# guanlongzhao/fac-via-ppg

Measured on AMD Instinct MI355X. Metric: 22.05 kHz audio samples/sec end-to-end PPG→wav; real-time factor at batch=1, higher is better.
Workload: dtype f32

## Files before the change

### fac-via-ppg_amd/csrc/facppg_taco.hip

```cpp

#include <algorithm>
#include <cstdlib>
#include <cstring>
#include <mutex>
#include <new>

#include "facppg_gemm.h"

using namespace facppg;

struct facppg_taco {
  facppg_taco_config c;
  int device;
  int coop_limit;
  int wall_khz;
  char* arena;
  float4 *pre0, *pre1, *conv[8], *wih;
  float *conv_b[8], *conv_scale[8], *conv_shift[8];
  float *whh_t[2], *lstm_b;
  float4* mem_w;
  float *dp0_t, *dp1_t, *att_t, *att_b, *dec_t, *dec_b, *q_t, *proj_t, *proj_b;
  float *loc_conv, *loc_dense, *v;
  float *att_coop[5], *dec_coop[5];
  int coop_U[5], coop_nwg[5];
// ... 976 lines not shown
  if (tid < U && unit0 + tid < A) {
    const float* gs = part + 4 * NT;
    const float h = lstm_point(gs[tid], gs[U + tid], gs[2 * U + tid], gs[3 * U + tid], &cstate[tid]);
    __hip_atomic_store(xchg_out + unit0 + tid, ((unsigned long long)tag << 32) | __float_as_uint(h), __ATOMIC_RELAXED,
                       __HIP_MEMORY_SCOPE_AGENT);
  }
}

template <int NT>
__device__ __forceinline__ void coop_gather(const unsigned long long* xchg, unsigned tag, int n, float* dst0, float* dst1, int tid) {
  for (int i = tid; i < n; i += NT) {
    const float h = __uint_as_float((unsigned)poll_tag(xchg + i, tag));
    dst0[i] = h; dst1[i] = h;
  }
  __syncthreads();
}

__global__ __launch_bounds__(NTC) void k_decoder_coop(DecArgs p) {
  extern __shared__ float sm[];
  __shared__ int s_stop;
  __shared__ float c_att[160], c_dec[160];
  const int wg = blockIdx.x, b = p.b0 + blockIdx.y, tid = threadIdx.x;
  const bool leader = wg == 0;
  const int len = p.lengths ? p.lengths[b] : p.Tin;
  DecLds L;
  dec_carve(p, sm, L);
  dec_init<NTC>(p, L, sm, tid);
  if (tid == 0) s_stop = 0;
  if (tid < 160) { c_att[tid] = 0.0f; c_dec[tid] = 0.0f; }
  __syncthreads();
  const float* mem = p.memory + (size_t)b * p.Tin * p.E;
  const float* pm = p.pm + (size_t)b * p.Tin * p.AD;
  float* ah = L.in_att + p.P + p.E;
  float* dh = L.in_dec + p.A + p.E;
  unsigned long long* xa = p.xchg + (size_t)b * 2 * p.A;
  unsigned long long* xd = xa + p.A;
  const int SC = 4 * p.U, unit0 = wg * p.U;
  const float* att_slice = p.att_coop + (size_t)wg * L.KA * SC;
  const float* dec_slice = p.dec_coop + (size_t)wg * L.KD * SC;
  long long tk = clock64();
#define PROF(slot)                                                        \
  if (p.prof && leader && b == 0 && tid == 0) {                           \
    const long long now = clock64();                                      \
    p.prof[slot] += now - tk;                                             \
    tk = now;                                                             \
  }
  for (int t = 0;; ++t) {
    if (t > 0) {
      dec_project<NTC>(p, L, t - 1, b, tid, leader, &s_stop);
      if (s_stop) {
        if (leader && tid == 0) p.out_len[b] = t;
        break;
      }
    }
    PROF(0)
    dec_prenet<NTC>(p, L, t, b, tid);
    PROF(1)
    coop_lstm_slice<NTC>(att_slice, p.att_b, L.KA, p.U, p.A, unit0, L.in_att, L.part, c_att, xa, t + 1, tid);
    PROF(2)
    coop_gather<NTC>(xa, t + 1, p.A, ah, L.in_dec, tid);
    PROF(3)
    PROF(4)
    dec_attention<NTC>(p, L, mem, pm, len, t, b, tid, leader);
    PROF(5)
    coop_lstm_slice<NTC>(dec_slice, p.dec_b, L.KD, p.U, p.D, unit0, L.in_dec, L.part, c_dec, xd, t + 1, tid);
    PROF(6)
    coop_gather<NTC>(xd, t + 1, p.D, dh, L.in_proj, tid);
    PROF(7)
  }
#undef PROF
}

constexpr int SU = 4, SSC = 4 * SU, SKP = NTC / SSC;
constexpr int SKR_LSTM = 40, SKR_PROJ = 32, SKR_P1 = 4, SKR_P2 = 12;

__device__ __forceinline__ void xpub(unsigned long long* w, float v, unsigned tag) {
  __hip_atomic_store(w, ((unsigned long long)tag << 32) | __float_as_uint(v), __ATOMIC_RELAXED, __HIP_MEMORY_SCOPE_AGENT);
}
__device__ __forceinline__ float xwait(const unsigned long long* w, unsigned tag) {
  return __uint_as_float((unsigned)poll_tag(w, tag));
}

template <int KRM>
__device__ __forceinline__ void stat_load(float (&w)[KRM], const float* __restrict__ W, int ld, int row0, int nrows, int K, int tid) {
  const int r = tid % SSC, kp = tid / SSC, KR = (K + SKP - 1) / SKP;
#pragma unroll
  for (int i = 0; i < KRM; ++i) {
    const int k = kp * KR + i;
    w[i] = (i < KR && k < K && row0 + r < nrows) ? W[(size_t)k * ld + row0 + r] : 0.0f;
  }
}
template <int KRM>
__device__ __forceinline__ void stat_mv16(const float (&w)[KRM], int K, const float* in, float* part, int tid) {
  const int r = tid % SSC, kp = tid / SSC, KR = (K + SKP - 1) / SKP;
  const int kb = kp * KR;
  float acc = 0.0f;
#pragma unroll
  for (int i = 0; i < KRM; ++i) acc = fmaf(w[i], in[kb + i], acc);
  acc += __shfl_xor(acc, 16);
  acc += __shfl_xor(acc, 32);
  if ((tid & 63) < SSC) part[(tid >> 6) * SSC + r] = acc;
  __syncthreads();
  if (tid < SSC) {
    float s = 0.0f;
#pragma unroll
    for (int j = 0; j < NTC / 64; ++j) s += part[j * SSC + tid];
    part[256 + tid] = s;
  }
  __syncthreads();
}

constexpr int SNU = 4;

template <int KRM, int NU>
__device__ __forceinline__ void stat_mv16n(const float (&w)[KRM], int K, const float* in0, int ustride, unsigned alive, float* part,
                                           int tid) {
  if constexpr (NU > 2) {
#pragma unroll
    for (int u = 0; u < NU; ++u)
      if (alive >> u & 1) {
        stat_mv16(w, K, in0 + (size_t)u * ustride, part, tid);
        if (tid < SSC) part[512 + u * SSC + tid] = part[256 + tid];
      }
    return;
  }
  const int r = tid % SSC, kp = tid / SSC, KR = (K + SKP - 1) / SKP;
  const int kb = kp * KR;
  float acc[NU];
#pragma unroll
  for (int u = 0; u < NU; ++u) acc[u] = 0.0f;
#pragma unroll
  for (int i = 0; i < KRM; ++i)
#pragma unroll
    for (int u = 0; u < NU; ++u) acc[u] = fmaf(w[i], in0[(size_t)u * ustride + kb + i], acc[u]);
#pragma unroll
  for (int u = 0; u < NU; ++u) {
    acc[u] += __shfl_xor(acc[u], 16);
    acc[u] += __shfl_xor(acc[u], 32);
    if ((tid & 63) < SSC) part[((tid >> 6) * NU + u) * SSC + r] = acc[u];
  }
  __syncthreads();
  if (tid < SSC * NU) {
    const int u = tid / SSC, rr = tid % SSC;
    float s = 0.0f;
#pragma unroll
    for (int j = 0; j < NTC / 64; ++j) s += part[(j * NU + u) * SSC + rr];
    part[512 + tid] = s;
  }
  __syncthreads();
  (void)alive;
}

template <int NU>
__global__ __launch_bounds__(NTC) void k_decoder_split(DecArgs p) {
  extern __shared__ float sm[];
  __shared__ int s_stop[SNU];
  __shared__ float c_att[SNU][SU], c_dec[SNU][SU];
  const int blk = blockIdx.x, grp = blockIdx.y, tid = threadIdx.x;
  const size_t xstride = (size_t)(p.NF + 1 + 2 * p.P + p.A + p.E + p.D + 8);
  const int KA = p.P + p.E + p.A, KD = p.A + p.E + p.D, KP = p.D + p.E;
  if (tid < SNU) s_stop[tid] = 0;
  if (blk >= NU) {
    const int wg = blk - NU, unit0 = wg * SU, row0 = wg * SSC;
    const int ustride = KA + KD + KP + round_up(p.NF, 4) + round_up(p.P, 4);
    float* part = sm + (size_t)NU * ustride;
    for (int i = tid; i < NU * ustride + 1024; i += NTC) sm[i] = 0.0f;
    if (tid < SNU * SU) { (&c_att[0][0])[tid] = 0.0f; (&c_dec[0][0])[tid] = 0.0f; }
    float w_att[SKR_LSTM], w_dec[SKR_LSTM], w_proj[SKR_PROJ], w_p1[SKR_PROJ], w_p2[SKR_P2];
    stat_load(w_att, p.att_w4 + (size_t)wg * KA * SSC, SSC, 0, SSC, KA, tid);
    stat_load(w_dec, p.dec_w4 + (size_t)wg * KD * SSC, SSC, 0, SSC, KD, tid);
    const int pre_wk = (p.P + SSC - 1) / SSC, proj_wk = (p.NF + 1 + SSC - 1) / SSC;
    const int proj_w0 = pre_wk + proj_wk <= p.nwk ? pre_wk : 0;
    const int prow0 = (wg - proj_w0) * SSC;
    stat_load(w_proj, p.proj_t, round_up(p.NF + 1, 4), prow0 < 0 ? p.NF + 1 : prow0, p.NF + 1, KP, tid);
    stat_load(w_p1, p.w1p_t, round_up(p.P, 4), row0, p.P, KP, tid);
    stat_load(w_p2, p.dp1_t, round_up(p.P, 4), row0, p.P, p.P, tid);
    const bool has_proj = prow0 >= 0 && prow0 < p.NF + 1, has_pre = row0 < p.P;
    unsigned alive = 0;
    for (int u = 0; u < NU; ++u)
      if (grp * NU + u < p.B) alive |= 1u << u;
    __syncthreads();
#define FOR_ALIVE(u) _Pragma("unroll") for (int u = 0; u < NU; ++u) if (alive >> u & 1)
#define UTT(u)                                                                                          \
  const int b = grp * NU + u;                                                                           \
  unsigned long long* MEL = p.xsplit + (size_t)b * xstride;                                             \
  unsigned long long *X1 = MEL + p.NF + 1, *X2 = X1 + p.P, *AH = X2 + p.P, *CTX = AH + p.A, *DH = CTX + p.E; \
  float* in_att = sm + (size_t)u * ustride; float* in_dec = in_att + KA; float* in_proj = in_dec + KD;  \
  float* xin = in_proj + KP; float* p1 = xin + round_up(p.NF, 4);                                       \
  (void)MEL; (void)X1; (void)X2; (void)AH; (void)CTX; (void)DH; (void)in_att; (void)in_dec; (void)in_proj; (void)xin; (void)p1
    long long wtk = clock64();
#define WPROF(slot)                                                       \
  if (p.prof && wg == 0 && grp == 0 && tid == 0) {                        \
    const long long now = clock64();                                      \
    p.prof[16 + slot] += now - wtk;                                       \
    wtk = now;                                                            \
  }
    for (int t = 0;; ++t) {
      const unsigned tag = t + 1;
      if (t > 0) {
        if (has_proj) stat_mv16n<SKR_PROJ, NU>(w_proj, KP, sm + KA + KD, ustride, alive, part, tid);
        if (has_proj) FOR_ALIVE(u) {
          UTT(u);
          if (tid < SSC && prow0 + tid <= p.NF) {
            const int row = prow0 + tid;
            const float v = part[512 + u * SSC + tid] + p.proj_b[row];
            if (row < p.NF) {
              p.mel[((size_t)b * p.NF + row) * p.max_steps + t - 1] = v;
              if (p.melx) xpub(p.melx + (size_t)(t - 1) * p.NF + row, v, tag - 1);
            } else { p.gate[(size_t)b * p.max_steps + t - 1] = v; xpub(MEL + row, v, tag); }
          }
        }
        if (has_pre) stat_mv16n<SKR_PROJ, NU>(w_p1, KP, sm + KA + KD, ustride, alive, part, tid);
        if (has_pre) FOR_ALIVE(u) {
          UTT(u);
          const uint8_t* mk = p.masks + ((size_t)t * 2 * p.B + b) * p.P;
          if (tid < SSC && row0 + tid < p.P)
            xpub(X1 + row0 + tid, fmaxf(part[512 + u * SSC + tid] + p.b1p[row0 + tid], 0.0f) * (float)mk[row0 + tid] * 2.0f, tag);
        }
        WPROF(0)
        FOR_ALIVE(u) {
          UTT(u);
          if (tid == 0) s_stop[u] = sigm(xwait(MEL + p.NF, tag)) > p.gate_thr || t == dec_step_limit(p, b);
        }
        __syncthreads();
        for (int u = 0; u < NU; ++u)
          if (s_stop[u]) alive &= ~(1u << u);
        if (!alive) break;
        FOR_ALIVE(u) {
          UTT(u);
          for (int i = tid; i < p.P; i += NTC) p1[i] = xwait(X1 + i, tag);
        }
        __syncthreads();
        WPROF(1)
      }
      if (has_pre) stat_mv16n<SKR_P2, NU>(w_p2, p.P, sm + KA + KD + KP + round_up(p.NF, 4), ustride, alive, part, tid);
      if (has_pre) FOR_ALIVE(u) {
        UTT(u);
        const uint8_t* mk = p.masks + ((size_t)t * 2 * p.B + b) * p.P;
        if (tid < SSC && row0 + tid < p.P)
          xpub(X2 + row0 + tid, fmaxf(part[512 + u * SSC + tid], 0.0f) * (float)mk[(size_t)p.B * p.P + row0 + tid] * 2.0f, tag);
      }
      WPROF(2)
      FOR_ALIVE(u) {
        UTT(u);
        for (int i = tid; i < p.P; i += NTC) in_att[i] = xwait(X2 + i, tag);
// ... 271 lines not shown
  auto take = [&](size_t bytes) { size_t o = off; off += (bytes + 255) / 256 * 256; return o; };
  const size_t E = c.encoder_embedding_dim > c.symbols_embedding_dim ? c.encoder_embedding_dim : c.symbols_embedding_dim;
  w.a0 = take((size_t)B * E * Tin * 4);
  w.a1 = take((size_t)B * E * Tin * 4);
  w.xproj = take((size_t)B * Tin * 4 * c.encoder_embedding_dim * 4);
  w.mem_cm = take((size_t)B * c.encoder_embedding_dim * Tin * 4);
  w.mask = take((size_t)2 * B * c.symbols_embedding_dim * Tin);
  w.xchg = take((size_t)B * 2 * 2 * (c.encoder_embedding_dim / 2) * 8);
  const size_t mx = c.encoder_embedding_dim > c.symbols_embedding_dim ? c.encoder_embedding_dim : c.symbols_embedding_dim;
  w.splitk_bytes = (size_t)16 * B * mx * Tin * 4;
  w.splitk = take(w.splitk_bytes);
  w.total = off;
  return w;
}

}

static int taco_check(const facppg_taco_config* c) {
  FACPPG_REQUIRE(c, FACPPG_EINVAL, "config is NULL");
  FACPPG_REQUIRE(c->n_symbols > 0 && c->symbols_embedding_dim > 0 && c->encoder_embedding_dim > 0 && c->encoder_embedding_dim % 2 == 0,
                 FACPPG_EINVAL, "bad encoder dims");
  FACPPG_REQUIRE(c->symbols_embedding_dim == c->encoder_embedding_dim, FACPPG_EUNSUPPORTED,
                 "symbols_embedding_dim must equal encoder_embedding_dim (prenet feeds the conv bank)");
  FACPPG_REQUIRE(c->encoder_n_convolutions >= 0 && c->encoder_n_convolutions <= 8 && c->postnet_n_convolutions >= 2 &&
                     c->postnet_n_convolutions <= 8 && c->encoder_kernel_size % 2 == 1 && c->postnet_kernel_size % 2 == 1,
                 FACPPG_EUNSUPPORTED, "conv stack sizes out of range");
  FACPPG_REQUIRE(c->attention_rnn_dim == c->decoder_rnn_dim && c->attention_rnn_dim % 4 == 0 && 4 * c->attention_rnn_dim <= 4096,
                 FACPPG_EUNSUPPORTED, "attention_rnn_dim must equal decoder_rnn_dim, be a multiple of 4 and <= 1024");
  FACPPG_REQUIRE(c->attention_location_n_filters >= 1 && c->attention_location_n_filters <= 32 && c->attention_dim >= 1 &&
                     c->attention_dim <= 256,
                 FACPPG_EUNSUPPORTED, "attention_location_n_filters must be <= 32 and attention_dim <= 256 (one MFMA pass each)");
  FACPPG_REQUIRE(c->encoder_embedding_dim <= 768 && c->prenet_dim <= NTC && c->attention_dim <= NTC && c->n_acoustic_feat_dims < NTC &&
                     (2 * c->encoder_embedding_dim) % 4 == 0,
                 FACPPG_EUNSUPPORTED, "decoder dims exceed the 512-thread cooperative workgroup");
  FACPPG_REQUIRE(c->attention_location_kernel_size % 2 == 1 && c->attention_location_n_filters > 0, FACPPG_EUNSUPPORTED,
                 "attention_location_kernel_size must be odd");
  return FACPPG_OK;
}

static size_t taco_count(const facppg_taco_config* c) {
  const size_t S = c->symbols_embedding_dim, E = c->encoder_embedding_dim, H = E / 2, K = c->encoder_kernel_size;
  const size_t P = c->prenet_dim, A = c->attention_rnn_dim, D = c->decoder_rnn_dim, AD = c->attention_dim, NF = c->n_acoustic_feat_dims;
  size_t n = S * c->n_symbols + S * S;
  n += (size_t)c->encoder_n_convolutions * (E * E * K + 5 * E);
  n += 2 * (4 * H * E + 4 * H * H + 8 * H);
  n += P * NF + P * P;
  n += 4 * A * (P + E) + 4 * A * A + 8 * A;
  n += AD * A + AD * E + AD + (size_t)c->attention_location_n_filters * 2 * c->attention_location_kernel_size +
       AD * c->attention_location_n_filters;
  n += 4 * D * (A + E) + 4 * D * D + 8 * D;
  n += NF * (D + E) + NF + (D + E) + 1;
  const size_t PE = c->postnet_embedding_dim, PK = c->postnet_kernel_size;
  for (int j = 0; j < c->postnet_n_convolutions; ++j) {
    const size_t ci = j == 0 ? NF : PE, co = j == c->postnet_n_convolutions - 1 ? NF : PE;
    n += co * ci * PK + 5 * co;
  }
  return n;
}

extern "C" size_t facppg_taco_weight_count(const facppg_taco_config* c) {
  if (taco_check(c) != FACPPG_OK) return 0;
  return taco_count(c);
}

extern "C" int facppg_taco_create(const facppg_taco_config* cfg, const float* wsrc, size_t n_floats, int device, void* stream_,
                                  facppg_taco** out) {
  if (int rc = taco_check(cfg)) return rc;
  FACPPG_REQUIRE(wsrc && out, FACPPG_EINVAL, "NULL argument");
  FACPPG_REQUIRE(n_floats == taco_count(cfg), FACPPG_EINVAL, "weight blob has %zu floats, expected %zu", n_floats, taco_count(cfg));
  hipStream_t s = (hipStream_t)stream_;
  FACPPG_HIP_CHECK(hipSetDevice(device));
  int n_cu = 0;
  FACPPG_HIP_CHECK(hipDeviceGetAttribute(&n_cu, hipDeviceAttributeMultiprocessorCount, device));
  facppg_taco* h = new (std::nothrow) facppg_taco();
  FACPPG_REQUIRE(h, FACPPG_EINVAL, "out of host memory");
  struct Guard {
    facppg_taco* h;
    ~Guard() { if (h) { if (h->arena) (void)hipFree(h->arena); delete h; } }
  } guard{h};
  h->c = *cfg; h->device = device;
  {
    int per_cu = 1;
    const struct { const void* fn; size_t lds; } coop_kernels[] = {
        {(const void*)k_decoder_coop, 150 * 1024}, {(const void*)k_decoder_forced<false>, 150 * 1024}, {(const void*)k_decoder_forced<true>, 150 * 1024}, {(const void*)k_decoder_split<1>, 150 * 1024},
        {(const void*)k_decoder_split<2>, 150 * 1024}, {(const void*)k_decoder_split<3>, 150 * 1024},
        {(const void*)k_bilstm_coop<32, 96, true>, 0}, {(const void*)k_bilstm_coop<64, 152, true>, 0},
        {(const void*)k_bilstm_coop<32, 96, false>, 0}, {(const void*)k_bilstm_coop<64, 152, false>, 0}};
    for (const auto& k : coop_kernels) {
      int nb = 0;
      if (k.lds) FACPPG_HIP_CHECK(hipFuncSetAttribute(k.fn, hipFuncAttributeMaxDynamicSharedMemorySize, (int)k.lds));
      FACPPG_HIP_CHECK(hipOccupancyMaxActiveBlocksPerMultiprocessor(&nb, k.fn, NTC, k.lds));
      per_cu = std::min(per_cu, nb);
    }
    const int resident = n_cu * per_cu;
    h->coop_limit = resident - resident / 16;
    static std::mutex poll_mu;
    static unsigned long long poll_devices = 0;
    {
      std::lock_guard<std::mutex> lock(poll_mu);
      const bool known = device < 64 && ((poll_devices >> device) & 1ull);
      if (!known) {
        const char* pl = getenv("FACPPG_POLL_LIMIT");
        const double seconds = pl ? strtod(pl, nullptr) : 20.0;
        int khz = 0;
        FACPPG_HIP_CHECK(hipDeviceGetAttribute(&khz, hipDeviceAttributeWallClockRate, device));
        const unsigned long long ticks = seconds > 0 && khz > 0 ? (unsigned long long)(seconds * 1e3 * khz) : 0ull;
        FACPPG_HIP_CHECK(hipMemcpyToSymbol(HIP_SYMBOL(g_poll_limit_ticks), &ticks, sizeof(ticks)));
        if (device < 64) poll_devices |= 1ull << device;
      }
    }
  }
  (void)hipDeviceGetAttribute(&h->wall_khz, hipDeviceAttributeWallClockRate, device);
  const facppg_taco_config& c = *cfg;
  const int S = c.symbols_embedding_dim, E = c.encoder_embedding_dim, H = E / 2, K = c.encoder_kernel_size;
  const int P = c.prenet_dim, A = c.attention_rnn_dim, D = c.decoder_rnn_dim, AD = c.attention_dim, NF = c.n_acoustic_feat_dims;
  const int NFIL = c.attention_location_n_filters, KSZ = c.attention_location_kernel_size;
  const int PE = c.postnet_embedding_dim, PK = c.postnet_kernel_size;
  const int Pp = round_up(P, 4), ADp = round_up(AD, 4), NFp = round_up(NF + 1, 4), G = 4 * A;

  size_t off = 0;
  auto take = [&](size_t bytes) { size_t o = off; off += (bytes + 255) / 256 * 256; return o; };
  struct { size_t pre0, pre1, conv[8], conv_b[8], conv_sc[8], conv_sh[8], wih, whh[2], lstm_b, mem_w, dp0, dp1, att, att_b, dec, dec_b, q,
           proj, proj_b, lc, ld, v, attc[5], decc[5], att4, dec4, w1p, b1p, post[8], post_b[8], post_sc[8], post_sh[8],
           tf_dp0, tf_dp1, tf_attx, tf_proj; } o;
  o.pre0 = take(packed_a_float4s(S, c.n_symbols) * 16);
  o.pre1 = take(packed_a_float4s(S, S) * 16);
  for (int j = 0; j < c.encoder_n_convolutions; ++j) {
    o.conv[j] = take(packed_a_float4s(E, E * K) * 16);
    o.conv_b[j] = take(E * 4); o.conv_sc[j] = take(E * 4); o.conv_sh[j] = take(E * 4);
  }
  o.wih = take(packed_a_float4s(8 * H, E) * 16);
  o.whh[0] = take((size_t)H * 4 * H * 4); o.whh[1] = take((size_t)H * 4 * H * 4);
  o.lstm_b = take((size_t)8 * H * 4);
  o.mem_w = take(packed_a_float4s(AD, E) * 16);
  o.dp0 = take((size_t)NF * Pp * 4); o.dp1 = take((size_t)P * Pp * 4);
  o.att = take((size_t)(P + E + A) * G * 4); o.att_b = take((size_t)G * 4);
  o.dec = take((size_t)(A + E + D) * G * 4); o.dec_b = take((size_t)G * 4);
  o.q = take((size_t)A * ADp * 4);
  o.proj = take((size_t)(D + E) * NFp * 4); o.proj_b = take((size_t)NFp * 4);
  const int CUs[5] = {8, 20, 40, 75, 150};
  for (int v = 0; v < 5; ++v) {
    const int nwg = (A + CUs[v] - 1) / CUs[v];
    o.attc[v] = take((size_t)nwg * (P + E + A) * 4 * CUs[v] * 4); o.decc[v] = take((size_t)nwg * (A + E + D) * 4 * CUs[v] * 4);
  }
  const int nwk = (A + 3) / 4;
  o.att4 = take((size_t)nwk * (P + E + A) * 16 * 4); o.dec4 = take((size_t)nwk * (A + E + D) * 16 * 4);
  o.w1p = take((size_t)(D + E) * Pp * 4); o.b1p = take((size_t)Pp * 4);
  o.lc = take((size_t)NFIL * 2 * KSZ * 4); o.ld = take((size_t)AD * NFIL * 4); o.v = take((size_t)AD * 4);
  for (int j = 0; j < c.postnet_n_convolutions; ++j) {
    const int ci = j == 0 ? NF : PE, co = j == c.postnet_n_convolutions - 1 ? NF : PE;
    o.post[j] = take(packed_a_float4s(co, ci * PK) * 16);
    o.post_b[j] = take(co * 4); o.post_sc[j] = take(co * 4); o.post_sh[j] = take(co * 4);
  }
  o.tf_dp0 = take(packed_a_float4s(P, NF) * 16); o.tf_dp1 = take(packed_a_float4s(P, P) * 16);
  o.tf_attx = take(packed_a_float4s(G, P) * 16); o.tf_proj = take(packed_a_float4s(NF + 1, D + E) * 16);
  if (hipMalloc((void**)&h->arena, off) != hipSuccess) {
    h->arena = nullptr;
    set_error("hipMalloc(%zu) failed", off);
    return FACPPG_EHIP;
  }
  int rc = FACPPG_OK;
  auto F = [&](size_t x) { return (float*)(h->arena + x); };
  auto F4 = [&](size_t x) { return (float4*)(h->arena + x); };
  auto hipok = [&](hipError_t e) { if (e != hipSuccess && !rc) { set_error("HIP error in facppg_taco_create: %s", hipGetErrorString(e)); rc = FACPPG_EHIP; } };
  auto cpy = [&](float* dst, const float* src, size_t n) { hipok(hipMemcpyAsync(dst, src, n * 4, hipMemcpyDeviceToDevice, s)); };
  auto tr = [&](const float* src, float* dst, int R, int Kk, int Rp, int k_off) {
    const int n = Kk * Rp;
    k_transpose_pad<<<(n + 255) / 256, 256, 0, s>>>(src, dst, R, Kk, Rp, k_off);
// ... 242 lines not shown
  attn_window_range(window, t, lengths[b], &lo, &hi);
  for (int q = blockIdx.x * blockDim.x + threadIdx.x; q < Tmax; q += gridDim.x * blockDim.x)
    mask[(size_t)b * Tmax + q] = (q >= lo && q <= hi) ? 0 : 1;
}
}

extern "C" int facppg_attention_window_mask(const int32_t* lengths_dev, int B, int Tmax, int window, int time_step,
                                            uint8_t* mask_dev, void* stream) {
  FACPPG_REQUIRE(lengths_dev && mask_dev, FACPPG_EINVAL, "NULL argument");
  FACPPG_REQUIRE(B > 0 && Tmax > 0 && B <= 65535 && time_step >= 0, FACPPG_EINVAL, "bad sizes B=%d Tmax=%d t=%d", B, Tmax, time_step);
  k_window_mask<<<dim3((Tmax + 255) / 256, B), 256, 0, (hipStream_t)stream>>>(lengths_dev, B, Tmax, window, time_step, mask_dev);
  FACPPG_HIP_CHECK(hipGetLastError());
  return FACPPG_OK;
}

extern "C" int facppg_taco_decode(const facppg_taco* h, const float* memory_dev, const float* pm_dev, const int32_t* lengths_dev,
                                  const int32_t* step_limits_dev, const uint8_t* masks_dev, uint64_t seed, int B, int Tin, int max_steps, float* mel_dev,
                                  float* gate_dev, float* align_dev, int32_t* out_lengths_dev, void* ws_, size_t ws_bytes,
                                  facppg_taco_decode_opts* opts, void* stream_) {
  FACPPG_REQUIRE(h && memory_dev && pm_dev && mel_dev && gate_dev && out_lengths_dev && ws_, FACPPG_EINVAL, "NULL argument");
  FACPPG_REQUIRE(B > 0 && Tin > 0 && max_steps > 0, FACPPG_EINVAL, "bad B/Tin/max_steps");
  FACPPG_REQUIRE(!opts || (opts->max_workgroups >= 0 && opts->frame_words_frames >= 0), FACPPG_EINVAL, "negative max_workgroups / frame_words_frames");
  FACPPG_REQUIRE(Tin <= 8192, FACPPG_EUNSUPPORTED, "Tin > 8192 does not fit the decoder's LDS state");
  const facppg_taco_config& c = h->c;
  hipStream_t s = (hipStream_t)stream_;
  const DecWs w = dec_ws(c, B, max_steps);
  FACPPG_REQUIRE(ws_bytes >= w.total, FACPPG_EWORKSPACE, "decode workspace has %zu bytes, need %zu", ws_bytes, w.total);
  char* ws = (char*)ws_;
  const uint8_t* masks = masks_dev;
  const size_t nmask = (size_t)max_steps * 2 * B * c.prenet_dim;
  if (!masks) {
    k_random_mask<<<(unsigned)((nmask + 255) / 256), 256, 0, s>>>((uint8_t*)(ws + w.mask), nmask, seed ^ 0xD1B54A32D192ED03ull);
    masks = (const uint8_t*)(ws + w.mask);
  }
  DecArgs a;
  a.melx = nullptr;
  a.dp0_t = h->dp0_t; a.dp1_t = h->dp1_t; a.att_t = h->att_t; a.att_b = h->att_b; a.dec_t = h->dec_t; a.dec_b = h->dec_b;
  a.q_t = h->q_t; a.proj_t = h->proj_t; a.proj_b = h->proj_b; a.loc_conv = h->loc_conv; a.loc_dense = h->loc_dense; a.v = h->v;
  a.xchg = (unsigned long long*)(ws + w.xchg);
  a.prof = getenv("FACPPG_DECODER_PROF") ? (long long*)(ws + w.prof) : nullptr;
  a.memory = memory_dev; a.pm = pm_dev; a.lengths = lengths_dev; a.step_limits = step_limits_dev; a.masks = masks; a.mel = mel_dev; a.gate = gate_dev;
  a.align = align_dev; a.out_len = out_lengths_dev;
  a.B = B; a.Tin = Tin; a.E = c.encoder_embedding_dim; a.P = c.prenet_dim; a.A = c.attention_rnn_dim; a.D = c.decoder_rnn_dim;
  a.AD = c.attention_dim; a.NF = c.n_acoustic_feat_dims; a.NFIL = c.attention_location_n_filters;
  a.KSZ = c.attention_location_kernel_size; a.window = c.attention_window_size; a.max_steps = max_steps;
  a.gate_thr = c.gate_threshold;
  const size_t smem = dec_lds_floats(a.P, a.E, a.A, a.D, a.NF, a.AD, a.NFIL, a.KSZ, Tin) * 4;
  FACPPG_REQUIRE(smem <= 160 * 1024 - 1024, FACPPG_EUNSUPPORTED, "decoder state (%zu bytes) exceeds LDS", smem);
  const int max_wgs = opts ? opts->max_workgroups : 0;
  const int wg_limit = max_wgs > 0 && max_wgs < h->coop_limit ? max_wgs : h->coop_limit;
  int launch_mode = 0, launch_wgs = B;
  const char* mode = getenv("FACPPG_DECODER_MODE");
  int variant = -1;
  const char* force_u = getenv("FACPPG_DECODER_COOP_U");
  for (int v = 0; v < 5 && variant < 0; ++v)
    if ((long)B * h->coop_nwg[v] <= wg_limit && (!force_u || atoi(force_u) == h->coop_U[v])) variant = v;
  int chunk = B;
  if (variant < 0 && !force_u && wg_limit / h->coop_nwg[4] >= 1) { variant = 4; chunk = wg_limit / h->coop_nwg[4]; }
  bool coop = variant >= 0;
  if (mode && !strcmp(mode, "single")) coop = false;
  if (mode && !strcmp(mode, "coop")) FACPPG_REQUIRE(coop, FACPPG_EUNSUPPORTED, "coop decoder needs B <= 120");
  if (coop) {
    a.att_coop = h->att_coop[variant]; a.dec_coop = h->dec_coop[variant]; a.U = h->coop_U[variant];
  }
  static const char* no_split = getenv("FACPPG_DECODER_NO_SPLIT");
  const char* max_nu_env = getenv("FACPPG_DECODER_SPLIT_MAX_NU");
  const int max_nu = max_nu_env ? atoi(max_nu_env) : 3;
  const size_t ustride = (size_t)(a.P + a.E + a.A) + (a.A + a.E + a.D) + (a.D + a.E) + round_up(a.NF, 4) + round_up(a.P, 4);
  int NU = 0;
  for (int nu = 1; nu <= SNU && nu <= max_nu && !NU; ++nu)
    if ((long)((B + nu - 1) / nu) * (h->split_nwk + nu) <= wg_limit && (nu * ustride + 1024) * 4 <= 150 * 1024) NU = nu;
  const bool split = coop && !no_split && NU > 0 && a.P + a.E + a.A <= SKP * SKR_LSTM &&
                     a.A + a.E + a.D <= SKP * SKR_LSTM && a.D + a.E <= SKP * SKR_PROJ && a.NF <= SKP * SKR_P1 &&
                     a.P <= SKP * SKR_P2 && a.NF + 1 <= h->split_nwk * SSC && a.P <= h->split_nwk * SSC &&
                     !(mode && !strcmp(mode, "coop"));
  if (mode && !strcmp(mode, "split")) FACPPG_REQUIRE(split, FACPPG_EUNSUPPORTED, "split decoder needs a small batch and the reference's layer widths");
  if (split) {
    a.att_w4 = h->att_w4; a.dec_w4 = h->dec_w4; a.xsplit = (unsigned long long*)(ws + w.xsplit);
    a.w1p_t = h->w1p_t; a.b1p = h->b1p;
    FACPPG_HIP_CHECK(hipMemsetAsync(ws + w.xchg, 0, w.total - w.xchg, s));
    size_t ssm = (NU * ustride + 1024) * 4;
    const size_t main_smem = (round_up((int)(smem / 4), 4) + (size_t)8 * NTC * 4) * 4;
    if (ssm < main_smem) ssm = main_smem;
    const void* fn = NU == 1 ? (const void*)k_decoder_split<1> : NU == 2 ? (const void*)k_decoder_split<2>
                   : NU == 3 ? (const void*)k_decoder_split<3> : (const void*)k_decoder_split<4>;
    FACPPG_HIP_CHECK(hipFuncSetAttribute(fn, hipFuncAttributeMaxDynamicSharedMemorySize, (int)ssm));
    void* args[] = {(void*)&a};
    const int groups = (B + NU - 1) / NU;
    a.nwk = h->split_nwk;
    unsigned long long* words = opts ? (unsigned long long*)opts->frame_words_dev : nullptr;
    a.melx = (B == 1 && words && opts->frame_words_frames >= max_steps) ? words : nullptr;
    a.dbg_flags = getenv("FACPPG_DECODER_NO_ROWS") ? 1 : 0;
    FACPPG_HIP_CHECK(launch_coop(fn, dim3(h->split_nwk + NU, groups), dim3(NTC), args, ssm, s));
    launch_mode = 2; launch_wgs = (h->split_nwk + NU) * groups;
    if (a.prof) {
      long long pr[32];
      FACPPG_HIP_CHECK(hipMemcpyAsync(pr, a.prof, sizeof(pr), hipMemcpyDeviceToHost, s));
      FACPPG_HIP_CHECK(hipStreamSynchronize(s));
      fprintf(stderr, "[facppg split decoder prof (main), shader cycles] location features %lld energy_pre %lld entering row %lld query weights requested %lld wait_gate %lld wait_ah %lld attention %lld | att: query %lld energy %lld softmax %lld update %lld context %lld\n",
              pr[6], pr[7], pr[14], pr[2], pr[0], pr[3], pr[5], pr[8], pr[10], pr[11], pr[12], pr[13]);
      fprintf(stderr, "[facppg split decoder prof (worker 0), shader cycles] proj+prenet1 %lld | gather gate,X1 %lld | prenet2 %lld | gather X2 %lld | "
              "att LSTM %lld | gather AH %lld | gather CTX %lld | dec LSTM + gather DH %lld | barrier %lld\n",
              pr[16], pr[17], pr[18], pr[19], pr[20], pr[21], pr[22], pr[23], pr[24]);
    }
  } else
  if (coop) {
    FACPPG_HIP_CHECK(hipMemsetAsync(ws + w.xchg, 0, w.total - w.xchg, s));
    const void* fn = (const void*)k_decoder_coop;
    FACPPG_HIP_CHECK(hipFuncSetAttribute(fn, hipFuncAttributeMaxDynamicSharedMemorySize, (int)smem));
    for (int b0 = 0; b0 < B; b0 += chunk) {
      const int nb = B - b0 < chunk ? B - b0 : chunk;
      int cv = variant;
      if (!force_u)
        for (int v = 0; v < variant; ++v)
          if ((long)nb * h->coop_nwg[v] <= wg_limit) { cv = v; break; }
      a.b0 = b0; a.att_coop = h->att_coop[cv]; a.dec_coop = h->dec_coop[cv]; a.U = h->coop_U[cv];
      void* args[] = {(void*)&a};
      FACPPG_HIP_CHECK(launch_coop(fn, dim3(h->coop_nwg[cv], nb), dim3(NTC), args, smem, s));
      launch_mode = 1; launch_wgs = h->coop_nwg[cv] * nb;
    }
    if (a.prof) {
      long long pr[16];
      FACPPG_HIP_CHECK(hipMemcpyAsync(pr, a.prof, sizeof(pr), hipMemcpyDeviceToHost, s));
      FACPPG_HIP_CHECK(hipStreamSynchronize(s));
      fprintf(stderr, "[facppg decoder prof, shader cycles] project %lld prenet %lld att_slice %lld sync1 %lld gather %lld attention %lld dec_slice %lld sync2 %lld | att: query %lld feat %lld energy %lld softmax %lld update %lld context %lld\n",
              pr[0], pr[1], pr[2], pr[3], pr[4], pr[5], pr[6], pr[7], pr[8], pr[9], pr[10], pr[11], pr[12], pr[13]);
    }
  } else {
    FACPPG_HIP_CHECK(hipFuncSetAttribute((const void*)k_decoder, hipFuncAttributeMaxDynamicSharedMemorySize, (int)smem));
    k_decoder<<<B, NT, smem, s>>>(a);
  }
  FACPPG_HIP_CHECK(hipGetLastError());
  if (opts) { opts->mode = launch_mode; opts->workgroups = launch_wgs; opts->streamed = a.melx != nullptr; }
  return FACPPG_OK;
}

namespace {
struct ForcedWs { size_t x0, p1, p2, xa, hc, mg, mask, xchg, prof, splitk, splitk_bytes, total; };
ForcedWs forced_ws(const facppg_taco_config& c, int B, int T) {
  ForcedWs w;
  size_t off = 0;
  auto take = [&](size_t bytes) { size_t o = off; off += (bytes + 255) / 256 * 256; return o; };
  const size_t BT = (size_t)B * T;
  w.x0 = take(BT * c.n_acoustic_feat_dims * 4);
  w.p1 = take(BT * c.prenet_dim * 4);
  w.p2 = take(BT * c.prenet_dim * 4);
  w.xa = take(BT * 4 * c.attention_rnn_dim * 4);
  w.hc = take(BT * (c.decoder_rnn_dim + c.encoder_embedding_dim) * 4);
  w.mg = take(BT * (c.n_acoustic_feat_dims + 1) * 4);
  w.mask = take(2 * BT * c.prenet_dim);
  w.xchg = take(BT * (c.attention_rnn_dim + c.encoder_embedding_dim + c.decoder_rnn_dim) * 8);
  w.prof = take(32 * 8);
  w.splitk_bytes = 16 * BT * (c.n_acoustic_feat_dims + 1) * 4;
  w.splitk = take(w.splitk_bytes);
  w.total = off;
  return w;
}
}

extern "C" size_t facppg_taco_decode_forced_workspace_bytes(const facppg_taco* h, int B, int T_out) {
  if (!h || B <= 0 || T_out <= 0) return 0;
  return forced_ws(h->c, B, T_out).total;
}

extern "C" int facppg_taco_draw_dropout_forced(const facppg_taco* h, const uint64_t* seeds_dev, int B, int T_out,
                                               uint8_t* dec_masks_dev, void* stream_) {
  FACPPG_REQUIRE(h && seeds_dev && dec_masks_dev, FACPPG_EINVAL, "NULL argument");
  FACPPG_REQUIRE(B > 0 && T_out > 0, FACPPG_EINVAL, "bad B/T_out");
  const size_t n = (size_t)2 * B * h->c.prenet_dim * T_out;
  k_random_mask_forced_utt<<<(unsigned)((n + 255) / 256), 256, 0, (hipStream_t)stream_>>>(dec_masks_dev, seeds_dev, B, h->c.prenet_dim, T_out);
  FACPPG_HIP_CHECK(hipGetLastError());
  return FACPPG_OK;
}

extern "C" int facppg_taco_decode_forced(const facppg_taco* h, const float* memory_dev, const float* pm_dev, const int32_t* lengths_dev,
// ... 284 lines not shown
```

Baseline: 4.638 million.

## Add fast split-decoder worker step with padded LDS layout and wave-level reductions

Adds a new worker path for the split decoder, used when NU is 1 or 2, that remaps threads so each wave's 32-lane halves each own one output row. Input vectors are stored in shared memory in a padded per-K-part layout, so each lane reads its stretch with float4 loads. The per-row sum is reduced inside the wave using DPP lane moves and readlane rather than the cross-wave shared-memory reduction of the old path. This is meant to cut LDS traffic and barriers in each decoder timestep. The cost is a more complex index mapping and a guard against register spills for NU>2, with the old path kept behind an environment variable.

```diff
diff --git a/fac-via-ppg_amd/csrc/facppg_taco.hip b/fac-via-ppg_amd/csrc/facppg_taco.hip
--- a/fac-via-ppg_amd/csrc/facppg_taco.hip
+++ b/fac-via-ppg_amd/csrc/facppg_taco.hip
@@ -1082,13 +1082,17 @@
 }
 
 template <int KRM>
-__device__ __forceinline__ void stat_load(float (&w)[KRM], const float* __restrict__ W, int ld, int row0, int nrows, int K, int tid) {
-  const int r = tid % SSC, kp = tid / SSC, KR = (K + SKP - 1) / SKP;
+__device__ __forceinline__ void stat_load_rk(float (&w)[KRM], const float* __restrict__ W, int ld, int row0, int nrows, int K, int r, int kp) {
+  const int KR = (K + SKP - 1) / SKP;
 #pragma unroll
   for (int i = 0; i < KRM; ++i) {
     const int k = kp * KR + i;
     w[i] = (i < KR && k < K && row0 + r < nrows) ? W[(size_t)k * ld + row0 + r] : 0.0f;
   }
+}
+template <int KRM>
+__device__ __forceinline__ void stat_load(float (&w)[KRM], const float* __restrict__ W, int ld, int row0, int nrows, int K, int tid) {
+  stat_load_rk(w, W, ld, row0, nrows, K, tid % SSC, tid / SSC);
 }
 template <int KRM>
 __device__ __forceinline__ void stat_mv16(const float (&w)[KRM], int K, const float* in, float* part, int tid) {
@@ -1151,9 +1155,242 @@
   (void)alive;
 }
 
+constexpr int fs_stride(int krm) { return (krm / 4) % 2 ? krm : krm + 4; }
+constexpr int FS_LSTM = fs_stride(SKR_LSTM), FS_PROJ = fs_stride(SKR_PROJ), FS_P2 = fs_stride(SKR_P2);
+constexpr int FS_USTRIDE = SKP * (2 * FS_LSTM + FS_PROJ + FS_P2);
+static_assert(SKR_LSTM % 4 == 0 && SKR_PROJ % 4 == 0 && SKR_P2 % 4 == 0, "float4 reads of a K part's stretch");
+
+struct FsLay { int KR, M; };
+__device__ __forceinline__ FsLay fs_lay(int K) { const int KR = (K + SKP - 1) / SKP; return {KR, (1 << 17) / KR + 1}; }
+template <int S>
+__device__ __forceinline__ int fs_pos(FsLay l, int k) { const int q = (k * l.M) >> 17; return q * S + (k - q * l.KR); }
+
+template <int KRM, int NU>
+__device__ __forceinline__ void fs_mv(const float (&w)[KRM], const float* in0, int kp, bool hi, float (&sum)[NU]) {
+  constexpr int S = fs_stride(KRM);
+  float acc[NU];
+#pragma unroll
+  for (int u = 0; u < NU; ++u) acc[u] = 0.0f;
+#pragma unroll
+  for (int j = 0; j < KRM / 4; ++j)
+#pragma unroll
+    for (int u = 0; u < NU; ++u) {
+      const float4 h4 = reinterpret_cast<const float4*>(in0 + (size_t)u * FS_USTRIDE + kp * S)[j];
+      acc[u] = fmaf(w[4 * j], h4.x, acc[u]); acc[u] = fmaf(w[4 * j + 1], h4.y, acc[u]);
+      acc[u] = fmaf(w[4 * j + 2], h4.z, acc[u]); acc[u] = fmaf(w[4 * j + 3], h4.w, acc[u]);
+    }
+#pragma unroll
+  for (int u = 0; u < NU; ++u) {
+    float a = acc[u];
+    a += lane_mov<0xB1>(a);
+    a += lane_mov<0x4E>(a);
+    float s0 = 0.0f, s1 = 0.0f;
+#pragma unroll
+    for (int j = 0; j < SKP / 4; ++j) {
+      s0 += __int_as_float(__builtin_amdgcn_readlane(__float_as_int(a), 4 * j));
+      s1 += __int_as_float(__builtin_amdgcn_readlane(__float_as_int(a), 32 + 4 * j));
+    }
+    sum[u] = hi ? s1 : s0;
+  }
+}
+
 template <int NU>
+__device__ __forceinline__ void split_worker_fast(const DecArgs& p, float* sm, int* s_stop, float (*c_att)[SU], float (*c_dec)[SU]) {
+  static_assert(NU <= 2, "three accumulator sets next to the weight registers spill");
+  const int blk = blockIdx.x, grp = blockIdx.y, tid = threadIdx.x;
+  const size_t xstride = (size_t)(p.NF + 1 + 2 * p.P + p.A + p.E + p.D + 8);
+  const int KA = p.P + p.E + p.A, KD = p.A + p.E + p.D, KP = p.D + p.E;
+  const int wg = blk - NU, unit0 = wg * SU, row0 = wg * SSC;
+  const int lane = tid & 63, wv = tid >> 6, kp = lane & 31;
+  const bool hi = lane >= 32, head = kp == 0;
+  const int r = (2 * (wv & 1) + (hi ? 1 : 0)) * SU + (wv >> 1);
+  float* part = sm + (size_t)NU * FS_USTRIDE;
+  for (int i = tid; i < NU * FS_USTRIDE + 1024; i += NTC) sm[i] = 0.0f;
+  if (tid < SNU * SU) { (&c_att[0][0])[tid] = 0.0f; (&c_dec[0][0])[tid] = 0.0f; }
+  const FsLay la = fs_lay(KA), ld = fs_lay(KD), lp = fs_lay(KP), l2 = fs_lay(p.P);
+  float w_att[SKR_LSTM], w_dec[SKR_LSTM], w_proj[SKR_PROJ], w_p1[SKR_PROJ], w_p2[SKR_P2];
+  stat_load_rk(w_att, p.att_w4 + (size_t)wg * KA * SSC, SSC, 0, SSC, KA, r, kp);
+  stat_load_rk(w_dec, p.dec_w4 + (size_t)wg * KD * SSC, SSC, 0, SSC, KD, r, kp);
+  const int pre_wk = (p.P + SSC - 1) / SSC, proj_wk = (p.NF + 1 + SSC - 1) / SSC;
+  const int proj_w0 = pre_wk + proj_wk <= p.nwk ? pre_wk : 0;
+  const int prow0 = (wg - proj_w0) * SSC;
+  stat_load_rk(w_proj, p.proj_t, round_up(p.NF + 1, 4), prow0 < 0 ? p.NF + 1 : prow0, p.NF + 1, KP, r, kp);
+  stat_load_rk(w_p1, p.w1p_t, round_up(p.P, 4), row0, p.P, KP, r, kp);
+  stat_load_rk(w_p2, p.dp1_t, round_up(p.P, 4), row0, p.P, p.P, r, kp);
+  const bool has_proj = prow0 >= 0 && prow0 < p.NF + 1, has_pre = row0 < p.P;
+  const int prow = prow0 + tid, qrow = row0 + tid, un = unit0 + r % SU, gate = r / SU;
+  const bool pub_proj = tid < SSC && has_proj && prow <= p.NF, pub_pre = tid < SSC && has_pre && qrow < p.P;
+  const float b_proj = pub_proj ? p.proj_b[prow] : 0.0f, b_p1 = pub_pre ? p.b1p[qrow] : 0.0f;
+  const float b_att = head && un < p.A ? p.att_b[gate * p.A + un] : 0.0f, b_dec = head && un < p.D ? p.dec_b[gate * p.D + un] : 0.0f;
+  unsigned alive = 0;
+  for (int u = 0; u < NU; ++u)
+    if (grp * NU + u < p.B) alive |= 1u << u;
+  __syncthreads();
+#define FOR_ALIVE(u) _Pragma("unroll") for (int u = 0; u < NU; ++u) if (alive >> u & 1)
+#define UTT(u)                                                                                          \
+  const int b = grp * NU + u;                                                                           \
+  unsigned long long* MEL = p.xsplit + (size_t)b * xstride;                                             \
+  unsigned long long *X1 = MEL + p.NF + 1, *X2 = X1 + p.P, *AH = X2 + p.P, *CTX = AH + p.A, *DH = CTX + p.E; \
+  float* in_att = sm + (size_t)u * FS_USTRIDE; float* in_dec = in_att + SKP * FS_LSTM; float* in_proj = in_dec + SKP * FS_LSTM; \
+  float* p1 = in_proj + SKP * FS_PROJ;                                                                  \
+  (void)MEL; (void)X1; (void)X2; (void)AH; (void)CTX; (void)DH; (void)in_att; (void)in_dec; (void)in_proj; (void)p1
+  long long wtk = clock64();
+#define WPROF(slot)                                                       \
+  if (p.prof && wg == 0 && grp == 0 && tid == 0) {                        \
+    const long long now = clock64();                                      \
+    p.prof[16 + slot] += now - wtk;                                       \
+    wtk = now;                                                            \
+  }
+  float sum[NU];
+  const size_t mframe = (size_t)2 * p.B * p.P;
+  unsigned nk1[NU], nk2[NU];
+#pragma unroll
+  for (int u = 0; u < NU; ++u) {
+    nk1[u] = 0; nk2[u] = 0;
+    if (pub_pre && (alive >> u & 1)) nk2[u] = p.masks[(size_t)(p.B + grp * NU + u) * p.P + qrow];
+  }
+  for (int t = 0;; ++t) {
+    const unsigned tag = t + 1;
+    unsigned k1[NU], k2[NU];
+#pragma unroll
+    for (int u = 0; u < NU; ++u) {
+      k1[u] = nk1[u]; k2[u] = nk2[u];
+      nk1[u] = 0; nk2[u] = 0;
+      if (pub_pre && (alive >> u & 1) && t + 1 < p.max_steps) {
+        const uint8_t* mk = p.masks + (size_t)(t + 1) * mframe + (size_t)(grp * NU + u) * p.P + qrow;
+        nk1[u] = mk[0]; nk2[u] = mk[(size_t)p.B * p.P];
+      }
+    }
+    if (t > 0) {
+      if (has_proj) {
+        fs_mv<SKR_PROJ, NU>(w_proj, sm + 2 * SKP * FS_LSTM, kp, hi, sum);
+        if (head)
+#pragma unroll
+          for (int u = 0; u < NU; ++u) part[(2 * NU + u) * SSC + r] = sum[u];
+      }
+      if (has_pre) {
+        fs_mv<SKR_PROJ, NU>(w_p1, sm + 2 * SKP * FS_LSTM, kp, hi, sum);
+        if (head)
+#pragma unroll
+          for (int u = 0; u < NU; ++u) part[(3 * NU + u) * SSC + r] = sum[u];
+      }
+      if (has_proj || has_pre) __syncthreads();
+      if (has_proj) {
+        FOR_ALIVE(u) {
+          UTT(u);
+          if (pub_proj) {
+            const float v = part[(2 * NU + u) * SSC + tid] + b_proj;
+            if (prow < p.NF) {
+              p.mel[((size_t)b * p.NF + prow) * p.max_steps + t - 1] = v;
+              if (p.melx) xpub(p.melx + (size_t)(t - 1) * p.NF + prow, v, tag - 1);
+            } else { p.gate[(size_t)b * p.max_steps + t - 1] = v; xpub(MEL + prow, v, tag); }
+          }
+        }
+      }
+      if (has_pre) {
+        FOR_ALIVE(u) {
+          UTT(u);
+          if (pub_pre) xpub(X1 + qrow, fmaxf(part[(3 * NU + u) * SSC + tid] + b_p1, 0.0f) * (float)k1[u] * 2.0f, tag);
+        }
+      }
+      WPROF(0)
+      FOR_ALIVE(u) {
+        UTT(u);
+        volatile int* flag = s_stop + u;
+        if (tid == NTC - 1) *flag = (int)(tag << 1) | (sigm(xwait(MEL + p.NF, tag)) > p.gate_thr || t == dec_step_limit(p, b) ? 1 : 0);
+        else if (tid < p.P) {
+          while ((*flag >> 1) != (int)tag) __builtin_amdgcn_s_sleep(1);
+          p1[fs_pos<FS_P2>(l2, tid)] = xwait(X1 + tid, tag);
+        }
+      }
+      __syncthreads();
+      for (int u = 0; u < NU; ++u)
+        if ((alive >> u & 1) && (s_stop[u] & 1)) alive &= ~(1u << u);
+      if (!alive) break;
+      WPROF(1)
+    }
+    if (has_pre) {
+      fs_mv<SKR_P2, NU>(w_p2, sm + SKP * (2 * FS_LSTM + FS_PROJ), kp, hi, sum);
+      if (head)
+#pragma unroll
+        for (int u = 0; u < NU; ++u) part[(4 * NU + u) * SSC + r] = sum[u];
+      __syncthreads();
+      FOR_ALIVE(u) {
+        UTT(u);
+        if (pub_pre) xpub(X2 + qrow, fmaxf(part[(4 * NU + u) * SSC + tid], 0.0f) * (float)k2[u] * 2.0f, tag);
+      }
+    }
+    WPROF(2)
+    FOR_ALIVE(u) {
+      UTT(u);
+      for (int i = tid; i < p.P; i += NTC) in_att[fs_pos<FS_LSTM>(la, i)] = xwait(X2 + i, tag);
+    }
+    __syncthreads();
+    WPROF(3)
+    fs_mv<SKR_LSTM, NU>(w_att, sm, kp, hi, sum);
+    if (head)
+#pragma unroll
+      for (int u = 0; u < NU; ++u) part[u * SSC + r] = sum[u] + b_att;
+    __syncthreads();
+    FOR_ALIVE(u) {
+      UTT(u);
+      if (tid < SU && unit0 + tid < p.A) {
+        const float* gs = part + u * SSC;
+        xpub(AH + unit0 + tid, lstm_point(gs[tid], gs[SU + tid], gs[2 * SU + tid], gs[3 * SU + tid], &c_att[u][tid]), tag);
+      }
+    }
+    WPROF(4)
+    FOR_ALIVE(u) {
+      UTT(u);
+      for (int i = tid; i < p.A; i += NTC) {
+        const int ia = fs_pos<FS_LSTM>(la, p.P + p.E + i), id = fs_pos<FS_LSTM>(ld, i);
+        const float h = xwait(AH + i, tag);
+        in_att[ia] = h; in_dec[id] = h;
+      }
+    }
+    WPROF(5)
+    FOR_ALIVE(u) {
+      UTT(u);
+      for (int i = tid; i < p.E; i += NTC) {
+        const int ia = fs_pos<FS_LSTM>(la, p.P + i), id = fs_pos<FS_LSTM>(ld, p.A + i), ip = fs_pos<FS_PROJ>(lp, p.D + i);
+        const float c = xwait(CTX + i, tag);
+        in_att[ia] = c; in_dec[id] = c; in_proj[ip] = c;
+      }
+    }
+    __syncthreads();
+    WPROF(6)
+    fs_mv<SKR_LSTM, NU>(w_dec, sm + SKP * FS_LSTM, kp, hi, sum);
+    if (head)
+#pragma unroll
+      for (int u = 0; u < NU; ++u) part[(NU + u) * SSC + r] = sum[u] + b_dec;
+    __syncthreads();
+    FOR_ALIVE(u) {
+      UTT(u);
+      if (tid < SU && unit0 + tid < p.D) {
+        const float* gs = part + (NU + u) * SSC;
+        xpub(DH + unit0 + tid, lstm_point(gs[tid], gs[SU + tid], gs[2 * SU + tid], gs[3 * SU + tid], &c_dec[u][tid]), tag);
+      }
+    }
+    FOR_ALIVE(u) {
+      UTT(u);
+      for (int i = tid; i < p.D; i += NTC) {
+        const int id = fs_pos<FS_LSTM>(ld, p.A + p.E + i), ip = fs_pos<FS_PROJ>(lp, i);
+        const float h = xwait(DH + i, tag);
+        in_dec[id] = h; in_proj[ip] = h;
+      }
+    }
+    WPROF(7)
+    __syncthreads();
+    WPROF(8)
+  }
+#undef WPROF
+#undef FOR_ALIVE
+#undef UTT
+}
+
+template <int NU, bool LEGACY>
 __global__ __launch_bounds__(NTC) void k_decoder_split(DecArgs p) {
-  extern __shared__ float sm[];
+  extern __shared__ __align__(16) float sm[];
   __shared__ int s_stop[SNU];
   __shared__ float c_att[SNU][SU], c_dec[SNU][SU];
   const int blk = blockIdx.x, grp = blockIdx.y, tid = threadIdx.x;
@@ -1161,6 +1398,10 @@
   const int KA = p.P + p.E + p.A, KD = p.A + p.E + p.D, KP = p.D + p.E;
   if (tid < SNU) s_stop[tid] = 0;
   if (blk >= NU) {
+    if constexpr (!LEGACY) {
+      split_worker_fast<NU>(p, sm, s_stop, c_att, c_dec);
+      return;
+    }
     const int wg = blk - NU, unit0 = wg * SU, row0 = wg * SSC;
     const int ustride = KA + KD + KP + round_up(p.NF, 4) + round_up(p.P, 4);
     float* part = sm + (size_t)NU * ustride;
@@ -1598,8 +1839,9 @@
   {
     int per_cu = 1;
     const struct { const void* fn; size_t lds; } coop_kernels[] = {
-        {(const void*)k_decoder_coop, 150 * 1024}, {(const void*)k_decoder_forced<false>, 150 * 1024}, {(const void*)k_decoder_forced<true>, 150 * 1024}, {(const void*)k_decoder_split<1>, 150 * 1024},
-        {(const void*)k_decoder_split<2>, 150 * 1024}, {(const void*)k_decoder_split<3>, 150 * 1024},
+        {(const void*)k_decoder_coop, 150 * 1024}, {(const void*)k_decoder_forced<false>, 150 * 1024}, {(const void*)k_decoder_forced<true>, 150 * 1024}, {(const void*)k_decoder_split<1, false>, 150 * 1024},
+        {(const void*)k_decoder_split<2, false>, 150 * 1024}, {(const void*)k_decoder_split<1, true>, 150 * 1024},
+        {(const void*)k_decoder_split<2, true>, 150 * 1024}, {(const void*)k_decoder_split<3, true>, 150 * 1024},
         {(const void*)k_bilstm_coop<32, 96, true>, 0}, {(const void*)k_bilstm_coop<64, 152, true>, 0},
         {(const void*)k_bilstm_coop<32, 96, false>, 0}, {(const void*)k_bilstm_coop<64, 152, false>, 0}};
     for (const auto& k : coop_kernels) {
@@ -2008,15 +2250,19 @@
     size_t ssm = (NU * ustride + 1024) * 4;
     const size_t main_smem = (round_up((int)(smem / 4), 4) + (size_t)8 * NTC * 4) * 4;
     if (ssm < main_smem) ssm = main_smem;
-    const void* fn = NU == 1 ? (const void*)k_decoder_split<1> : NU == 2 ? (const void*)k_decoder_split<2>
-                   : NU == 3 ? (const void*)k_decoder_split<3> : (const void*)k_decoder_split<4>;
+    const char* step_env = getenv("FACPPG_DECODER_STEP");
+    a.dbg_flags = (getenv("FACPPG_DECODER_NO_ROWS") ? 1 : 0) | (step_env && !strcmp(step_env, "legacy") ? 2 : 0);
+    const bool legacy_step = (a.dbg_flags & 2) || NU > 2;
+    if (!legacy_step && ssm < ((size_t)NU * FS_USTRIDE + 1024) * 4) ssm = ((size_t)NU * FS_USTRIDE + 1024) * 4;
+    const void* fn = !legacy_step ? (NU == 1 ? (const void*)k_decoder_split<1, false> : (const void*)k_decoder_split<2, false>)
+                   : NU == 1 ? (const void*)k_decoder_split<1, true> : NU == 2 ? (const void*)k_decoder_split<2, true>
+                   : NU == 3 ? (const void*)k_decoder_split<3, true> : (const void*)k_decoder_split<4, true>;
     FACPPG_HIP_CHECK(hipFuncSetAttribute(fn, hipFuncAttributeMaxDynamicSharedMemorySize, (int)ssm));
     void* args[] = {(void*)&a};
     const int groups = (B + NU - 1) / NU;
     a.nwk = h->split_nwk;
     unsigned long long* words = opts ? (unsigned long long*)opts->frame_words_dev : nullptr;
     a.melx = (B == 1 && words && opts->frame_words_frames >= max_steps) ? words : nullptr;
-    a.dbg_flags = getenv("FACPPG_DECODER_NO_ROWS") ? 1 : 0;
     FACPPG_HIP_CHECK(launch_coop(fn, dim3(h->split_nwk + NU, groups), dim3(NTC), args, ssm, s));
     launch_mode = 2; launch_wgs = (h->split_nwk + NU) * groups;
     if (a.prof) {
```

New measurement: 4.647 million, median of 3. No clear change (+0.2%).
